# google-research/big_vision

Hardware: NVIDIA H100
Metric: siglip_vit_b16_pairs_per_sec (higher is better)
Workload: dtype bf16

## Files before the change

big_vision_b200/csrc/common.cuh:

```cuda
#pragma once
#include <cuda.h>
#include <cuda_bf16.h>
#include <cuda_runtime.h>
#include <stdint.h>
#include "wgmma.cuh"

namespace bv {

typedef __nv_bfloat16 bf16;

enum : int { DT_F32 = 0, DT_BF16 = 1 };

__device__ __forceinline__ uint32_t smem_u32(const void* p) {
  return static_cast<uint32_t>(__cvta_generic_to_shared(p));
}
__device__ __forceinline__ uint32_t lane_id() { return threadIdx.x & 31; }

__device__ __forceinline__ uint32_t pin_reg(uint32_t v) {
  return __shfl_sync(0xffffffffu, v, static_cast<int>(threadIdx.x & 31));
}
__device__ __forceinline__ int pin_reg(int v) { return static_cast<int>(pin_reg(static_cast<uint32_t>(v))); }
__device__ __forceinline__ float pin_reg(float v) { return __uint_as_float(pin_reg(__float_as_uint(v))); }
template <typename T>
__device__ __forceinline__ T* pin_reg(T* v) {
  const unsigned long long u = reinterpret_cast<unsigned long long>(v);
  const uint32_t lo = pin_reg(static_cast<uint32_t>(u)), hi = pin_reg(static_cast<uint32_t>(u >> 32));
  return reinterpret_cast<T*>((static_cast<unsigned long long>(hi) << 32) | lo);
}

__device__ __forceinline__ float warp_sum(float v) {
#pragma unroll
  for (int o = 16; o > 0; o >>= 1) v += __shfl_xor_sync(0xffffffffu, v, o);
  return v;
}
__device__ __forceinline__ float warp_max(float v) {
#pragma unroll
  for (int o = 16; o > 0; o >>= 1) v = fmaxf(v, __shfl_xor_sync(0xffffffffu, v, o));
  return v;
}

__device__ __forceinline__ uint32_t pack_bf16(float lo, float hi) {
  __nv_bfloat162 v = __floats2bfloat162_rn(lo, hi);
  return *reinterpret_cast<uint32_t*>(&v);
}
__device__ __forceinline__ uint4 ld_nc_na(const uint4* p) {
  uint4 v;
  asm volatile("ld.global.nc.L1::no_allocate.v4.u32 {%0, %1, %2, %3}, [%4];"
               : "=r"(v.x), "=r"(v.y), "=r"(v.z), "=r"(v.w) : "l"(p));
  return v;
}
__device__ __forceinline__ float bf16_lo(uint32_t v) { return __uint_as_float(v << 16); }
__device__ __forceinline__ float bf16_hi(uint32_t v) { return __uint_as_float(v & 0xffff0000u); }
__device__ __forceinline__ float round_bf16(float x) {
  return __bfloat162float(__float2bfloat16_rn(x));
}

__device__ __forceinline__ float tanh_fast(float x) {
  float y;
  asm("tanh.approx.f32 %0, %1;" : "=f"(y) : "f"(x));
  return y;
}
__device__ __forceinline__ float gelu_tanh(float x) {
  const float k0 = 0.7978845608028654f, k1 = 0.044715f;
  float u = k0 * (x + k1 * x * x * x);
  float t = 1.0f - 2.0f / (1.0f + __expf(2.0f * u));
  return 0.5f * x * (1.0f + t);
}
__device__ __forceinline__ float gelu_tanh_grad(float x) {
  const float k0 = 0.7978845608028654f, k1 = 0.044715f;
  float x2 = x * x;
  float u = k0 * (x + k1 * x * x2);
  float t = 1.0f - 2.0f / (1.0f + __expf(2.0f * u));
  float du = k0 * (1.0f + 3.0f * k1 * x2);
  return 0.5f * (1.0f + t) + 0.5f * x * (1.0f - t * t) * du;
}

__device__ __forceinline__ float gelu_tanh_fast(float x) {
  const float k0 = 0.7978845608028654f, k01 = 0.7978845608028654f * 0.044715f;
  const float t = tanh_fast(x * fmaf(k01, x * x, k0));
  const float h = 0.5f * x;
  return fmaf(h, t, h);
}
__device__ __forceinline__ float gelu_tanh_grad_fast(float x) {
  const float k0 = 0.7978845608028654f, k01 = 0.7978845608028654f * 0.044715f;
  const float x2 = x * x;
  const float t = tanh_fast(x * fmaf(k01, x2, k0));
  const float du = fmaf(3.0f * k01, x2, k0);
  return fmaf(0.5f * x * fmaf(-t, t, 1.0f), du, fmaf(0.5f, t, 0.5f));
}

__device__ __forceinline__ void mbar_init(uint32_t bar, uint32_t count) {
  asm volatile("mbarrier.init.shared::cta.b64 [%0], %1;" ::"r"(bar), "r"(count) : "memory");
}
__device__ __forceinline__ void mbar_expect_tx(uint32_t bar, uint32_t bytes) {
  asm volatile("mbarrier.arrive.expect_tx.shared::cta.b64 _, [%0], %1;" ::"r"(bar), "r"(bytes)
               : "memory");
}
__device__ __forceinline__ void mbar_arrive(uint32_t bar) {
  asm volatile("mbarrier.arrive.shared::cta.b64 _, [%0];" ::"r"(bar) : "memory");
}
__device__ __forceinline__ void mbar_wait(uint32_t bar, uint32_t parity) {
  uint32_t ok;
  do {
#ifdef BV_MBAR_SUSPEND_NS
    asm volatile(
        "{\n"
        ".reg .pred p;\n"
        "mbarrier.try_wait.parity.shared::cta.b64 p, [%1], %2, %3;\n"
        "selp.u32 %0, 1, 0, p;\n"
        "}\n"
        : "=r"(ok)
        : "r"(bar), "r"(parity), "r"(static_cast<uint32_t>(BV_MBAR_SUSPEND_NS))
        : "memory");
#else
    asm volatile(
        "{\n"
        ".reg .pred p;\n"
        "mbarrier.try_wait.parity.shared::cta.b64 p, [%1], %2;\n"
        "selp.u32 %0, 1, 0, p;\n"
        "}\n"
        : "=r"(ok)
        : "r"(bar), "r"(parity)
        : "memory");
#endif
  } while (!ok);
}
__device__ __forceinline__ bool mbar_test(uint32_t bar, uint32_t parity) {
  uint32_t ok;
  asm volatile(
      "{\n"
      ".reg .pred p;\n"
      "mbarrier.test_wait.parity.shared::cta.b64 p, [%1], %2;\n"
      "selp.u32 %0, 1, 0, p;\n"
      "}\n"
      : "=r"(ok)
      : "r"(bar), "r"(parity)
      : "memory");
  return ok != 0;
}
__device__ __forceinline__ bool elect_one() {
  uint32_t pred;
  asm volatile(
      "{\n"
      ".reg .pred P;\n"
      "elect.sync _|P, 0xffffffff;\n"
      "selp.u32 %0, 1, 0, P;\n"
      "}\n"
      : "=r"(pred));
  return pred != 0;
}
__device__ __forceinline__ void fence_barrier_init() {
  asm volatile("fence.mbarrier_init.release.cluster;" ::: "memory");
}
__device__ __forceinline__ void fence_proxy_async() {
  asm volatile("fence.proxy.async.shared::cta;" ::: "memory");
}
__device__ __forceinline__ void named_bar_sync(uint32_t id, uint32_t nthreads) {
  asm volatile("bar.sync %0, %1;" ::"r"(id), "r"(nthreads) : "memory");
}

__device__ __forceinline__ void tma_prefetch_desc(const CUtensorMap* m) {
  asm volatile("prefetch.tensormap [%0];" ::"l"(reinterpret_cast<uint64_t>(m)) : "memory");
}
__device__ __forceinline__ void tma_load_2d(uint32_t dst, const CUtensorMap* m, uint32_t bar,
                                            int c0, int c1) {
  asm volatile(
      "cp.async.bulk.tensor.2d.shared::cluster.global.mbarrier::complete_tx::bytes"
      " [%0], [%1, {%3, %4}], [%2];"
      ::"r"(dst), "l"(reinterpret_cast<uint64_t>(m)), "r"(bar), "r"(c0), "r"(c1)
      : "memory");
}
__device__ __forceinline__ void tma_load_3d(uint32_t dst, const CUtensorMap* m, uint32_t bar,
                                            int c0, int c1, int c2) {
  asm volatile(
      "cp.async.bulk.tensor.3d.shared::cluster.global.mbarrier::complete_tx::bytes"
      " [%0], [%1, {%3, %4, %5}], [%2];"
      ::"r"(dst), "l"(reinterpret_cast<uint64_t>(m)), "r"(bar), "r"(c0), "r"(c1), "r"(c2)
      : "memory");
}
__device__ __forceinline__ void tma_load_4d(uint32_t dst, const CUtensorMap* m, uint32_t bar,
                                            int c0, int c1, int c2, int c3) {
  asm volatile(
      "cp.async.bulk.tensor.4d.shared::cluster.global.mbarrier::complete_tx::bytes"
      " [%0], [%1, {%3, %4, %5, %6}], [%2];"
      ::"r"(dst), "l"(reinterpret_cast<uint64_t>(m)), "r"(bar), "r"(c0), "r"(c1), "r"(c2), "r"(c3)
      : "memory");
}
__device__ __forceinline__ void tma_store_2d(const CUtensorMap* m, uint32_t src, int c0, int c1) {
  asm volatile("cp.async.bulk.tensor.2d.global.shared::cta.bulk_group [%0, {%2, %3}], [%1];"
               ::"l"(reinterpret_cast<uint64_t>(m)), "r"(src), "r"(c0), "r"(c1)
               : "memory");
}
__device__ __forceinline__ void tma_store_3d(const CUtensorMap* m, uint32_t src, int c0, int c1,
                                             int c2) {
  asm volatile("cp.async.bulk.tensor.3d.global.shared::cta.bulk_group [%0, {%2, %3, %4}], [%1];"
               ::"l"(reinterpret_cast<uint64_t>(m)), "r"(src), "r"(c0), "r"(c1), "r"(c2)
               : "memory");
}
__device__ __forceinline__ void tma_reduce_add_2d(const CUtensorMap* m, uint32_t src, int c0,
                                                  int c1) {
  asm volatile(
      "cp.reduce.async.bulk.tensor.2d.global.shared::cta.add.bulk_group [%0, {%2, %3}], [%1];"
      ::"l"(reinterpret_cast<uint64_t>(m)), "r"(src), "r"(c0), "r"(c1)
      : "memory");
}
__device__ __forceinline__ void tma_reduce_add_3d(const CUtensorMap* m, uint32_t src, int c0,
                                                  int c1, int c2) {
  asm volatile(
      "cp.reduce.async.bulk.tensor.3d.global.shared::cta.add.bulk_group [%0, {%2, %3, %4}], [%1];"
      ::"l"(reinterpret_cast<uint64_t>(m)), "r"(src), "r"(c0), "r"(c1), "r"(c2)
      : "memory");
}
__device__ __forceinline__ void tma_store_commit() {
  asm volatile("cp.async.bulk.commit_group;" ::: "memory");
}
template <int N>
__device__ __forceinline__ void tma_store_wait_read() {
  asm volatile("cp.async.bulk.wait_group.read %0;" ::"n"(N) : "memory");
}
template <int N>
__device__ __forceinline__ void tma_store_wait() {
  asm volatile("cp.async.bulk.wait_group %0;" ::"n"(N) : "memory");
}

}
```

big_vision_b200/csrc/gemm.cu:

```cuda
#include "common.cuh"
#include "gemm_sched.h"
#include "host_utils.h"

#include <atomic>

#include <stdlib.h>
#include <string.h>

namespace bv {

namespace {

constexpr int BM = 128;
constexpr int BK = 64;
constexpr int A_STAGE_BYTES = BM * BK * 2;
constexpr int NUM_THREADS = 384;
constexpr int SUB_BYTES = 64 * 64 * 2;

enum : int { EF_BIAS = 0, EF_GELU = 1, EF_RESID = 2, EF_DGELU = 3, EF_RESID_ROWMOD = 4, EF_GELU_ACT = 5 };
enum : int { OM_F32 = 0, OM_BF16_ADD = 1, OM_BF16_TMA = 2 };

template <int BN, int OM, int EF>
struct Cfg {
  static constexpr int B_STAGE_BYTES = BN * BK * 2;
  static constexpr int STAGE_BYTES = A_STAGE_BYTES + B_STAGE_BYTES;
  static constexpr bool AUX_TMA = OM == OM_BF16_TMA && (EF == EF_RESID || EF == EF_DGELU);
  static constexpr int OUTS = OM != OM_BF16_TMA ? 0 : (EF == EF_GELU ? 2 : 1);
  static constexpr int BUF_BYTES = OUTS * SUB_BYTES;
  static constexpr int BUFS = AUX_TMA ? BN / 64 : 2;
  static constexpr int STAGING_BYTES = 2 * BUFS * BUF_BYTES;
  static constexpr int SMEM_LIMIT = 232448 - 2048;
  static constexpr int STAGES_FIT = (SMEM_LIMIT - STAGING_BYTES) / STAGE_BYTES;
  static constexpr int STAGES = STAGES_FIT > 8 ? 8 : STAGES_FIT;
  static constexpr int STAGING_OFFSET = STAGES * STAGE_BYTES;
  static constexpr int BAR_OFFSET = STAGING_OFFSET + STAGING_BYTES;
  static constexpr int AUX_BAR = 2 * STAGES;
  static constexpr int SMEM_BYTES = BAR_OFFSET + 256 + 1024;
  static_assert(STAGES >= 3, "shared-memory budget leaves fewer than 3 stages");
  static_assert(8 * (AUX_BAR + (AUX_TMA ? 2 * BUFS : 0)) <= 256, "barriers overflow their 256 bytes");
};

struct GemmDev {
  GemmSched s;
  int M, N;
  int a_mn, b_mn;
  int reduce_out;
  float alpha;
  const float* bias;
  const bf16* aux;
  void* d; void* d2;
  long long ldd, ldd2, ldaux;
  float* colsum;
  int aux_row_mod;
};

template <int BN, int STAGES, int STAGE_BYTES, int TA, int TB, typename F>
__device__ __forceinline__ void mainloop(float (&acc)[BN / 2], uint32_t base, uint32_t bar_base, int cw,
                                         PipeState& ps, int kb0, int kb1, F&& after_first) {
  constexpr uint32_t a_lbo = TA ? 8192u : 16u, b_lbo = TB ? 8192u : 16u;
  constexpr uint32_t a_kstep = TA ? 2048u : 32u, b_kstep = TB ? 2048u : 32u;
  int prev_stage = -1;
  for (int kb = kb0; kb < kb1; ++kb) {
    mbar_wait(bar_base + 8u * ps.stage, ps.phase);
    const uint32_t a_s = base + ps.stage * STAGE_BYTES + cw * 8192;
    const uint32_t b_s = base + ps.stage * STAGE_BYTES + A_STAGE_BYTES;
    const uint64_t adesc = wgmma_desc_sw128(a_s, a_lbo, 1024u), bdesc = wgmma_desc_sw128(b_s, b_lbo, 1024u);
    wgmma_fence_regs(acc);
    wgmma_fence();
#pragma unroll
    for (int k = 0; k < BK / 16; ++k) {
      const uint64_t a = adesc + k * (a_kstep >> 4), b = bdesc + k * (b_kstep >> 4);
      const int accumulate = (kb > kb0 || k > 0) ? 1 : 0;
      if constexpr (BN == 256) wgmma_ss_n256<TA, TB>(acc, a, b, accumulate);
      else wgmma_ss_n128<TA, TB>(acc, a, b, accumulate);
    }
    wgmma_commit();
    wgmma_fence_regs(acc);
    if (kb == kb0) after_first();
    wgmma_wait<1>();
    if (prev_stage >= 0 && (threadIdx.x & 127) == 0) mbar_arrive(bar_base + 8u * (STAGES + prev_stage));
    prev_stage = ps.stage;
    ps.advance(STAGES);
  }
  wgmma_wait<0>();
  wgmma_fence_regs(acc);
  if (prev_stage >= 0 && (threadIdx.x & 127) == 0) mbar_arrive(bar_base + 8u * (STAGES + prev_stage));
}

__device__ __forceinline__ void aux_global(const GemmDev& p, int row, int col, bool pair, float& a0, float& a1) {
  const long long ar = p.aux_row_mod > 0 ? (row % p.aux_row_mod) : row;
  const bf16* ap = p.aux + ar * p.ldaux + col;
  if (pair) {
    const uint32_t q = *reinterpret_cast<const uint32_t*>(ap);
    a0 = bf16_lo(q); a1 = bf16_hi(q);
  } else {
    a0 = __bfloat162float(*ap);
    a1 = 0.f;
  }
}

template <bool OUT_F32, int EF>
__device__ __forceinline__ void epi_math(float alpha, float c0, float c1, float b0, float b1, float a0, float a1,
                                         float& v0, float& v1, float& pre0, float& pre1) {
  v0 = c0 * alpha + b0;
  v1 = c1 * alpha + b1;
  pre0 = pre1 = 0.f;
  if (EF == EF_GELU || EF == EF_GELU_ACT) {
    pre0 = round_bf16(v0); pre1 = round_bf16(v1);
    v0 = gelu_tanh_fast(pre0); v1 = gelu_tanh_fast(pre1);
  } else if (EF == EF_RESID || EF == EF_RESID_ROWMOD) {
    v0 = (OUT_F32 ? v0 : round_bf16(v0)) + a0;
    v1 = (OUT_F32 ? v1 : round_bf16(v1)) + a1;
  } else if (EF == EF_DGELU) {
    v0 *= gelu_tanh_grad_fast(a0);
    v1 *= gelu_tanh_grad_fast(a1);
  }
}


__device__ __forceinline__ void colsum_add(float* colsum, int N, float s0, float s1, int col, int lane) {
  s0 += __shfl_xor_sync(0xffffffffu, s0, 4);
  s0 += __shfl_xor_sync(0xffffffffu, s0, 8);
  s0 += __shfl_xor_sync(0xffffffffu, s0, 16);
  s1 += __shfl_xor_sync(0xffffffffu, s1, 4);
  s1 += __shfl_xor_sync(0xffffffffu, s1, 8);
  s1 += __shfl_xor_sync(0xffffffffu, s1, 16);
  if (lane < 4) {
    if (col < N) atomicAdd(colsum + col, s0);
    if (col + 1 < N) atomicAdd(colsum + col + 1, s1);
  }
}

template <int BN, bool OUT_F32, int EF>
__device__ __forceinline__ void epilogue_regs(const GemmDev& p, const float (&acc)[BN / 2], int m0, int n0,
                                              int cw, int kb0) {
  const int lane = threadIdx.x & 31, warp = (threadIdx.x >> 5) & 3;
  const int row0 = m0 + cw * 64 + warp * 16 + (lane >> 2);
  const int pM = p.M, pN = p.N;
  const float alpha = p.alpha;
  const bool reduce = p.reduce_out != 0;
  const bool first = kb0 == 0;
#pragma unroll
  for (int j = 0; j < BN / 8; ++j) {
    const int col = n0 + 8 * j + 2 * (lane & 3);
    if (col >= pN) continue;
    const bool pair = col + 1 < pN;
    float b0 = 0.f, b1 = 0.f;
    if (p.bias != nullptr && first) {
      b0 = __ldg(p.bias + col);
      if (pair) b1 = __ldg(p.bias + col + 1);
    }
#pragma unroll
    for (int h = 0; h < 2; ++h) {
      const int row = row0 + 8 * h;
      if (row >= pM) continue;
      float v0, v1, pre0, pre1, a0 = 0.f, a1 = 0.f;
      if ((EF == EF_RESID && first) || EF == EF_DGELU) aux_global(p, row, col, pair, a0, a1);
      epi_math<OUT_F32, EF>(alpha, acc[4 * j + 2 * h], acc[4 * j + 2 * h + 1], b0, b1, a0, a1, v0, v1, pre0, pre1);
      if (OUT_F32) {
        float* dp = static_cast<float*>(p.d) + row * p.ldd + col;
        if (reduce) {
          atomicAdd(dp, v0);
          if (pair) atomicAdd(dp + 1, v1);
        } else if (pair) {
          *reinterpret_cast<float2*>(dp) = make_float2(v0, v1);
        } else {
          *dp = v0;
        }
      } else {
        bf16* dp = static_cast<bf16*>(p.d) + row * p.ldd + col;
        const __nv_bfloat162 o = __floats2bfloat162_rn(v0, v1);
        if (pair) atomicAdd(reinterpret_cast<__nv_bfloat162*>(dp), o);
        else atomicAdd(dp, o.x);
      }
    }
  }
}

template <int BN, int EF, int BUF_BYTES>
__device__ __forceinline__ void epilogue_tma(const GemmDev& p, const CUtensorMap* tmD, const CUtensorMap* tmD2,
                                             const float (&acc)[BN / 2], int m0, int n0, int cw, uint32_t staging,
                                             uint32_t& nstore, uint32_t aux_bar, uint32_t aux_parity) {
  constexpr bool AUX_TMA = (EF == EF_RESID || EF == EF_DGELU);
  const int lane = threadIdx.x & 31, warp = (threadIdx.x >> 5) & 3;
  const bool leader = (threadIdx.x & 127) == 0;
  const int rl0 = warp * 16 + (lane >> 2);
  const int row0 = m0 + cw * 64 + rl0;
  const int pM = p.M, pN = p.N, pN8 = p.N & ~7;
  const float alpha = p.alpha;
#pragma unroll
  for (int c = 0; c < BN / 64; ++c) {
    uint32_t buf;
    if constexpr (AUX_TMA) {
      buf = staging + c * BUF_BYTES;
      mbar_wait(aux_bar + 8u * c, aux_parity);
    } else {
      buf = staging + (nstore & 1u) * BUF_BYTES;
      if (leader) tma_store_wait_read<1>();
      named_bar_sync(1 + cw, 128);
    }
    float cs[8][2];
#pragma unroll
    for (int jj = 0; jj < 8; ++jj) {
      const int j = 8 * c + jj;
      const int col = n0 + 8 * j + 2 * (lane & 3);
      cs[jj][0] = cs[jj][1] = 0.f;
      const bool cin = col < pN, pair = col + 1 < pN;
      float b0 = 0.f, b1 = 0.f;
      if (cin && p.bias != nullptr) {
        b0 = __ldg(p.bias + col);
        if (pair) b1 = __ldg(p.bias + col + 1);
      }
#pragma unroll
      for (int h = 0; h < 2; ++h) {
        const int rl = rl0 + 8 * h, row = row0 + 8 * h;
        const uint32_t off = rl * 128 + ((jj ^ (rl & 7)) << 4) + (lane & 3) * 4;
        float v0 = 0.f, v1 = 0.f, pre0 = 0.f, pre1 = 0.f;
        const bool in = cin && row < pM;
        if (in) {
          float a0 = 0.f, a1 = 0.f;
          if constexpr (AUX_TMA) {
            uint32_t q;
            asm volatile("ld.shared.b32 %0, [%1];" : "=r"(q) : "r"(buf + off));
            a0 = bf16_lo(q); a1 = bf16_hi(q);
          } else if constexpr (EF == EF_RESID_ROWMOD) {
            aux_global(p, row, col, pair, a0, a1);
          }
          epi_math<false, EF>(alpha, acc[4 * j + 2 * h], acc[4 * j + 2 * h + 1], b0, b1, a0, a1, v0, v1, pre0, pre1);
        }
        const __nv_bfloat162 o = __floats2bfloat162_rn(v0, v1);
        if (in) {
          cs[jj][0] += __low2float(o);
          cs[jj][1] += pair ? __high2float(o) : 0.f;
        }
        asm volatile("st.shared.b32 [%0], %1;" ::"r"(buf + off), "r"(*reinterpret_cast<const uint32_t*>(&o))
                     : "memory");
        if (EF == EF_GELU) {
          const __nv_bfloat162 q = __floats2bfloat162_rn(pre0, pre1);
          asm volatile("st.shared.b32 [%0], %1;" ::"r"(buf + SUB_BYTES + off),
                       "r"(*reinterpret_cast<const uint32_t*>(&q))
                       : "memory");
        }
      }
    }
    fence_proxy_async();
    named_bar_sync(1 + cw, 128);
    if (leader) {
      if (n0 + 64 * c < pN8 && m0 + cw * 64 < pM) {
        tma_store_2d(tmD, buf, n0 + 64 * c, m0 + cw * 64);
        if (EF == EF_GELU) tma_store_2d(tmD2, buf + SUB_BYTES, n0 + 64 * c, m0 + cw * 64);
      }
      tma_store_commit();
    }
    const int tail0 = pN8 - (n0 + 64 * c);
    if (pN8 < pN && tail0 >= 0 && tail0 < 64) {
      const int t = threadIdx.x & 127, rl = t & 63, out = t >> 6;
      const int row = m0 + cw * 64 + rl;
      if (row < pM && (out == 0 || EF == EF_GELU)) {
        const uint32_t src = buf + out * SUB_BYTES + rl * 128 + (((tail0 >> 3) ^ (rl & 7)) << 4);
        uint16_t* dst = reinterpret_cast<uint16_t*>(out ? p.d2 : p.d) + row * (out ? p.ldd2 : p.ldd) + pN8;
#pragma unroll 1
        for (int e = 0; e < pN - pN8; ++e) {
          uint16_t u;
          asm volatile("ld.shared.u16 %0, [%1];" : "=h"(u) : "r"(src + 2 * e));
          dst[e] = u;
        }
      }
      named_bar_sync(1 + cw, 128);
    }
    if (!AUX_TMA) ++nstore;
    if (p.colsum != nullptr) {
#pragma unroll
      for (int jj = 0; jj < 8; ++jj)
        colsum_add(p.colsum, pN, cs[jj][0], cs[jj][1], n0 + 8 * (8 * c + jj) + 2 * (lane & 3), lane);
    }
  }
}

template <int BN>
__device__ __forceinline__ void issue_aux_loads(const CUtensorMap* tmAux, int M, int N, int m0, int n0, int cw,
                                                uint32_t staging, uint32_t aux_bar) {
  tma_store_wait_read<0>();
#pragma unroll
  for (int c = 0; c < BN / 64; ++c) {
    const uint32_t bar = aux_bar + 8u * c;
    if (n0 + 64 * c < N && m0 + cw * 64 < M) {
      mbar_expect_tx(bar, SUB_BYTES);
      tma_load_2d(staging + c * SUB_BYTES, tmAux, bar, n0 + 64 * c, m0 + cw * 64);
    } else {
      mbar_arrive(bar);
    }
  }
}

template <int BN, int OM, int EF>
__global__ void __launch_bounds__(NUM_THREADS, 1)
gemm_kernel(const __grid_constant__ CUtensorMap tmA, const __grid_constant__ CUtensorMap tmB,
            const __grid_constant__ CUtensorMap tmD, const __grid_constant__ CUtensorMap tmD2,
            const __grid_constant__ CUtensorMap tmAux, const GemmDev p) {
  using C = Cfg<BN, OM, EF>;
  extern __shared__ uint8_t smem_raw[];
  const uint32_t raw_addr = smem_u32(smem_raw);
  const uint32_t base = (raw_addr + 1023u) & ~1023u;
  const uint32_t bar_base = base + C::BAR_OFFSET;
  auto full_bar = [&](int s) { return bar_base + 8u * s; };
  auto empty_bar = [&](int s) { return bar_base + 8u * (C::STAGES + s); };

  const int wg = __shfl_sync(0xffffffffu, static_cast<int>(threadIdx.x >> 7), 0);
  const int units = p.s.units;

  if (threadIdx.x == 0) {
    tma_prefetch_desc(&tmA);
    tma_prefetch_desc(&tmB);
    if (C::AUX_TMA) tma_prefetch_desc(&tmAux);
    for (int s = 0; s < C::STAGES; ++s) {
      mbar_init(full_bar(s), 1);
      mbar_init(empty_bar(s), 2);
    }
    if (C::AUX_TMA) {
      for (int b = 0; b < 2 * C::BUFS; ++b) mbar_init(bar_base + 8u * (C::AUX_BAR + b), 1);
    }
    fence_barrier_init();
  }
  __syncthreads();

  if (wg == 0) {
    asm volatile("setmaxnreg.dec.sync.aligned.u32 40;");
    if (threadIdx.x == 0) {
      PipeState ps;
      for (int u = blockIdx.x; u < units; u += gridDim.x) {
        const WorkUnit w = gemm_work_unit(p.s, u, BM, BN);
        for (int kb = w.kb0; kb < w.kb1; ++kb) {
          mbar_wait(empty_bar(ps.stage), ps.phase ^ 1u);
          const uint32_t a_s = base + ps.stage * C::STAGE_BYTES;
          const uint32_t b_s = a_s + A_STAGE_BYTES;
          const uint32_t fb = full_bar(ps.stage);
          mbar_expect_tx(fb, C::STAGE_BYTES);
          const int k0 = kb * BK;
          if (p.a_mn) {
#pragma unroll
            for (int j = 0; j < BM / 64; ++j) tma_load_2d(a_s + j * 8192, &tmA, fb, w.m0 + 64 * j, k0);
          } else {
            tma_load_2d(a_s, &tmA, fb, k0, w.m0);
          }
          if (p.b_mn) {
#pragma unroll
            for (int j = 0; j < BN / 64; ++j) tma_load_2d(b_s + j * 8192, &tmB, fb, w.n0 + 64 * j, k0);
          } else {
            tma_load_2d(b_s, &tmB, fb, k0, w.n0);
          }
          ps.advance(C::STAGES);
        }
      }
    }
    return;
  }

  asm volatile("setmaxnreg.inc.sync.aligned.u32 232;");
  const int cw = wg - 1;
  const uint32_t staging = base + C::STAGING_OFFSET + cw * C::BUFS * C::BUF_BYTES;
  const uint32_t aux_bar = bar_base + 8u * (C::AUX_BAR + cw * C::BUFS);
  const bool leader = (threadIdx.x & 127) == 0;
  uint32_t nstore = 0, nunit = 0;
  PipeState ps;
  constexpr int S = C::STAGES, SB = C::STAGE_BYTES;
  for (int u = blockIdx.x; u < units; u += gridDim.x, ++nunit) {
    const WorkUnit w = gemm_work_unit(p.s, u, BM, BN);
    auto after_first = [&]() {
      if constexpr (C::AUX_TMA) {
        if (leader) issue_aux_loads<BN>(&tmAux, p.M, p.N, w.m0, w.n0, cw, staging, aux_bar);
      }
    };
    float acc[BN / 2];
    if (p.a_mn) {
      if (p.b_mn) mainloop<BN, S, SB, 1, 1>(acc, base, bar_base, cw, ps, w.kb0, w.kb1, after_first);
      else mainloop<BN, S, SB, 1, 0>(acc, base, bar_base, cw, ps, w.kb0, w.kb1, after_first);
    } else {
      if (p.b_mn) mainloop<BN, S, SB, 0, 1>(acc, base, bar_base, cw, ps, w.kb0, w.kb1, after_first);
      else mainloop<BN, S, SB, 0, 0>(acc, base, bar_base, cw, ps, w.kb0, w.kb1, after_first);
    }

    if constexpr (OM == OM_BF16_TMA)
      epilogue_tma<BN, EF, C::BUF_BYTES>(p, &tmD, &tmD2, acc, w.m0, w.n0, cw, staging, nstore, aux_bar, nunit & 1u);
    else epilogue_regs<BN, OM == OM_F32, EF>(p, acc, w.m0, w.n0, cw, w.kb0);
  }
  if (OM == OM_BF16_TMA && (threadIdx.x & 127) == 0) tma_store_wait<0>();
}

template <int BN, int OM, int EF>
int launch_cfg(const bv_gemm_args& g, cudaStream_t stream) {
  using C = Cfg<BN, OM, EF>;
  CUtensorMap tmA, tmB, tmD, tmD2, tmAux;
  int rc;
  const CUtensorMapDataType bf = CU_TENSOR_MAP_DATA_TYPE_BFLOAT16;
  if (g.a_mn) rc = make_tmap_2d(&tmA, bf, g.A, g.M, g.K, g.lda * 2, 64, 64);
  else        rc = make_tmap_2d(&tmA, bf, g.A, g.K, g.M, g.lda * 2, 64, BM);
  if (rc) return rc;
  if (g.b_mn) rc = make_tmap_2d(&tmB, bf, g.B, g.N, g.K, g.ldb * 2, 64, 64);
  else        rc = make_tmap_2d(&tmB, bf, g.B, g.K, g.N, g.ldb * 2, 64, BN);
  if (rc) return rc;

  GemmDev p;
  const long long tiles = ((g.M + BM - 1) / BM) * ((g.N + BN - 1) / BN);
  if (tiles * ((g.K + BK - 1) / BK) > 0x7fffffffLL) { set_error("bv_gemm: problem too large"); return BV_ERR_INVALID; }
  if (!gemm_make_sched(g.M, g.N, g.K, BM, BN, BK, g.splits, g.reduce_out != 0, num_sms(), &p.s)) {
    set_error("bv_gemm: split-K requires reduce_out=1");
    return BV_ERR_INVALID;
  }
  p.M = (int)g.M; p.N = (int)g.N;
  p.a_mn = g.a_mn; p.b_mn = g.b_mn; p.reduce_out = g.reduce_out;
  p.alpha = g.alpha;
  p.bias = g.epilogue == BV_EPI_NONE ? nullptr : g.bias;
  p.colsum = g.colsum;
  p.aux = reinterpret_cast<const bf16*>(g.aux);
  p.ldaux = g.ldaux;
  p.aux_row_mod = g.aux_row_mod;
  p.d = g.D; p.d2 = g.D2;
  p.ldd = g.ldd; p.ldd2 = g.ldd2;
  memset(&tmD, 0, sizeof(tmD));
  memset(&tmD2, 0, sizeof(tmD2));
  memset(&tmAux, 0, sizeof(tmAux));
  const long long n8 = g.N & ~7LL;
  if (OM == OM_BF16_TMA && n8 > 0) {
    rc = make_tmap_2d(&tmD, bf, g.D, n8, g.M, g.ldd * 2, 64, 64);
    if (rc) return rc;
    if (EF == EF_GELU) {
      rc = make_tmap_2d(&tmD2, bf, g.D2, n8, g.M, g.ldd2 * 2, 64, 64);
      if (rc) return rc;
    }
  }
  if (C::AUX_TMA) {
    rc = make_tmap_2d(&tmAux, bf, g.aux, g.N, g.M, g.ldaux * 2, 64, 64);
    if (rc) return rc;
  }

  auto kern = gemm_kernel<BN, OM, EF>;
  static std::atomic<bool> attr_set[64];
  int dev = 0;
  if (cudaGetDevice(&dev) != cudaSuccess || dev < 0 || dev >= 64) dev = -1;
  if (dev < 0 || !attr_set[dev].load(std::memory_order_acquire)) {
    rc = check_cuda(cudaFuncSetAttribute(kern, cudaFuncAttributeMaxDynamicSharedMemorySize, C::SMEM_BYTES),
                    "cudaFuncSetAttribute(gemm)");
    if (rc) return rc;
    if (dev >= 0) attr_set[dev].store(true, std::memory_order_release);
  }
  const int grid = p.s.units < num_sms() ? p.s.units : num_sms();
  kern<<<grid, NUM_THREADS, C::SMEM_BYTES, stream>>>(tmA, tmB, tmD, tmD2, tmAux, p);
  return check_cuda(cudaGetLastError(), "gemm_kernel launch");
}

template <int BN>
int dispatch_epi(const bv_gemm_args& g, cudaStream_t s) {
  const bool f32 = (g.out_dtype == DT_F32), add = !f32 && g.reduce_out;
  switch (g.epilogue) {
    case BV_EPI_NONE:
    case BV_EPI_BIAS:
      return f32 ? launch_cfg<BN, OM_F32, EF_BIAS>(g, s)
                 : add ? launch_cfg<128, OM_BF16_ADD, EF_BIAS>(g, s) : launch_cfg<BN, OM_BF16_TMA, EF_BIAS>(g, s);
    case BV_EPI_BIAS_RESID:
      if (f32) return launch_cfg<BN, OM_F32, EF_RESID>(g, s);
      if (add) return launch_cfg<128, OM_BF16_ADD, EF_RESID>(g, s);
      return g.aux_row_mod > 0 ? launch_cfg<BN, OM_BF16_TMA, EF_RESID_ROWMOD>(g, s)
                               : launch_cfg<BN, OM_BF16_TMA, EF_RESID>(g, s);
    case BV_EPI_BIAS_GELU:
      return launch_cfg<BN, OM_BF16_TMA, EF_GELU>(g, s);
    case BV_EPI_BIAS_GELU_ACT:
      return launch_cfg<BN, OM_BF16_TMA, EF_GELU_ACT>(g, s);
    case BV_EPI_DGELU:
      if (f32) { set_error("bv_gemm: DGELU epilogue writes bf16"); return BV_ERR_INVALID; }
      if (g.aux_row_mod > 0) { set_error("bv_gemm: DGELU takes a row-aligned aux"); return BV_ERR_INVALID; }
      return add ? launch_cfg<128, OM_BF16_ADD, EF_DGELU>(g, s) : launch_cfg<BN, OM_BF16_TMA, EF_DGELU>(g, s);
  }
  set_error("bv_gemm: bad epilogue %d", g.epilogue);
  return BV_ERR_INVALID;
}

}
}

extern "C" {

int bv_gemm(const bv_gemm_args* args, void* stream) {
  using namespace bv;
  const cudaStream_t s = static_cast<cudaStream_t>(stream);
  if (!args) { set_error("bv_gemm: null args"); return BV_ERR_INVALID; }
  const bv_gemm_args& g = *args;
  if (g.M <= 0 || g.N <= 0 || g.K <= 0) { set_error("bv_gemm: empty problem"); return BV_ERR_INVALID; }
  if (g.out_dtype == DT_BF16 && ((reinterpret_cast<uintptr_t>(g.D) & 15) || (g.ldd % 8))) {
    set_error("bv_gemm: bf16 output must be 16B aligned with ldd %% 8 == 0"); return BV_ERR_INVALID;
  }
  if (g.out_dtype == DT_F32 && ((reinterpret_cast<uintptr_t>(g.D) & 7) || (g.ldd % 2))) {
    set_error("bv_gemm: fp32 output must be 8B aligned with an even ldd"); return BV_ERR_INVALID;
  }
  if (g.M > 0x7fffffffLL || g.N > 0x7fffffffLL || g.K > 0x7fffffffLL) {
    set_error("bv_gemm: dimension exceeds int32"); return BV_ERR_INVALID;
  }
  if (g.epilogue < BV_EPI_NONE || g.epilogue > BV_EPI_BIAS_GELU_ACT) {
    set_error("bv_gemm: bad epilogue %d", g.epilogue); return BV_ERR_INVALID;
  }
  if ((g.epilogue == BV_EPI_BIAS_RESID || g.epilogue == BV_EPI_DGELU) && g.aux == nullptr) {
    set_error("bv_gemm: epilogue %d needs aux", g.epilogue); return BV_ERR_INVALID;
  }
  if (g.aux != nullptr && ((reinterpret_cast<uintptr_t>(g.aux) & 15) || (g.ldaux % 8))) {
    set_error("bv_gemm: aux must be 16B aligned with ldaux %% 8 == 0"); return BV_ERR_INVALID;
  }
  if (g.bias != nullptr && (reinterpret_cast<uintptr_t>(g.bias) & 15)) {
    set_error("bv_gemm: bias must be 16B aligned"); return BV_ERR_INVALID;
  }
  if (g.epilogue == BV_EPI_BIAS_GELU && (g.out_dtype != DT_BF16 || g.D2 == nullptr || g.reduce_out)) {
    set_error("bv_gemm: BIAS_GELU needs bf16 output, D2 and no reduce"); return BV_ERR_INVALID;
  }
  if (g.epilogue == BV_EPI_BIAS_GELU && ((reinterpret_cast<uintptr_t>(g.D2) & 15) || (g.ldd2 % 8))) {
    set_error("bv_gemm: D2 must be 16B aligned with ldd2 %% 8 == 0"); return BV_ERR_INVALID;
  }
  if (g.epilogue == BV_EPI_BIAS_GELU_ACT && (g.out_dtype != DT_BF16 || g.reduce_out)) {
    set_error("bv_gemm: BIAS_GELU_ACT needs bf16 output and no reduce"); return BV_ERR_INVALID;
  }
  if (g.out_dtype != DT_F32 && g.out_dtype != DT_BF16) { set_error("bv_gemm: bad out dtype"); return BV_ERR_INVALID; }
  if (g.colsum != nullptr && (g.out_dtype != DT_BF16 || g.reduce_out)) {
    set_error("bv_gemm: colsum needs a plain bf16 output"); return BV_ERR_INVALID;
  }
  int bn = g.block_n;
  if (bn == 0) bn = (g.N > 128) ? 256 : 128;
  if (bn == 256) return dispatch_epi<256>(g, s);
  if (bn == 128) return dispatch_epi<128>(g, s);
  set_error("bv_gemm: block_n must be 0, 128 or 256");
  return BV_ERR_INVALID;
}

}
```

Measured before the change: 2765.

## Add ping-pong consumer schedule for TMA-stored GEMMs with small K

Adds a ping-pong mode where the two consumer warpgroups alternate whole 128x128 work units instead of splitting rows of one unit. Each warpgroup computes both 64-row halves, and named barriers order the mainloops so one group's epilogue overlaps the other's MMA. It is selected for bf16 TMA-output GEMMs with K<=1024, such as the ViT-B projections. The cost is a doubled accumulator register footprint, extra staging buffers for aux loads, and fixed BN=128 tiles in place of the chosen BN.

New measurement: 2825 (median of 6 runs). 1.02x the previous value.

```diff
diff --git a/big_vision_b200/csrc/common.cuh b/big_vision_b200/csrc/common.cuh
--- a/big_vision_b200/csrc/common.cuh
+++ b/big_vision_b200/csrc/common.cuh
@@ -158,6 +158,9 @@
 __device__ __forceinline__ void named_bar_sync(uint32_t id, uint32_t nthreads) {
   asm volatile("bar.sync %0, %1;" ::"r"(id), "r"(nthreads) : "memory");
 }
+__device__ __forceinline__ void named_bar_arrive(uint32_t id, uint32_t nthreads) {
+  asm volatile("bar.arrive %0, %1;" ::"r"(id), "r"(nthreads) : "memory");
+}
 
 __device__ __forceinline__ void tma_prefetch_desc(const CUtensorMap* m) {
   asm volatile("prefetch.tensormap [%0];" ::"l"(reinterpret_cast<uint64_t>(m)) : "memory");
diff --git a/big_vision_b200/csrc/gemm.cu b/big_vision_b200/csrc/gemm.cu
--- a/big_vision_b200/csrc/gemm.cu
+++ b/big_vision_b200/csrc/gemm.cu
@@ -16,18 +16,20 @@
 constexpr int A_STAGE_BYTES = BM * BK * 2;
 constexpr int NUM_THREADS = 384;
 constexpr int SUB_BYTES = 64 * 64 * 2;
+constexpr uint32_t ORDER_BAR = 3;
+constexpr long long PINGPONG_MAX_K = 1024;
 
 enum : int { EF_BIAS = 0, EF_GELU = 1, EF_RESID = 2, EF_DGELU = 3, EF_RESID_ROWMOD = 4, EF_GELU_ACT = 5 };
 enum : int { OM_F32 = 0, OM_BF16_ADD = 1, OM_BF16_TMA = 2 };
 
-template <int BN, int OM, int EF>
+template <int BN, int OM, int EF, bool PP>
 struct Cfg {
   static constexpr int B_STAGE_BYTES = BN * BK * 2;
   static constexpr int STAGE_BYTES = A_STAGE_BYTES + B_STAGE_BYTES;
   static constexpr bool AUX_TMA = OM == OM_BF16_TMA && (EF == EF_RESID || EF == EF_DGELU);
   static constexpr int OUTS = OM != OM_BF16_TMA ? 0 : (EF == EF_GELU ? 2 : 1);
   static constexpr int BUF_BYTES = OUTS * SUB_BYTES;
-  static constexpr int BUFS = AUX_TMA ? BN / 64 : 2;
+  static constexpr int BUFS = AUX_TMA ? (PP ? 2 : 1) * BN / 64 : 2;
   static constexpr int STAGING_BYTES = 2 * BUFS * BUF_BYTES;
   static constexpr int SMEM_LIMIT = 232448 - 2048;
   static constexpr int STAGES_FIT = (SMEM_LIMIT - STAGING_BYTES) / STAGE_BYTES;
@@ -54,36 +56,43 @@
   int aux_row_mod;
 };
 
-template <int BN, int STAGES, int STAGE_BYTES, int TA, int TB, typename F>
-__device__ __forceinline__ void mainloop(float (&acc)[BN / 2], uint32_t base, uint32_t bar_base, int cw,
-                                         PipeState& ps, int kb0, int kb1, F&& after_first) {
+template <int BN, int H, int STAGES, int STAGE_BYTES, int TA, int TB, typename F, typename G>
+__device__ __forceinline__ void mainloop(float (&acc)[H][BN / 2], uint32_t base, uint32_t bar_base, uint32_t a_off,
+                                         PipeState& ps, int kb0, int kb1, F&& after_first, G&& after_issue) {
   constexpr uint32_t a_lbo = TA ? 8192u : 16u, b_lbo = TB ? 8192u : 16u;
   constexpr uint32_t a_kstep = TA ? 2048u : 32u, b_kstep = TB ? 2048u : 32u;
   int prev_stage = -1;
   for (int kb = kb0; kb < kb1; ++kb) {
     mbar_wait(bar_base + 8u * ps.stage, ps.phase);
-    const uint32_t a_s = base + ps.stage * STAGE_BYTES + cw * 8192;
+    const uint32_t a_s = base + ps.stage * STAGE_BYTES + a_off;
     const uint32_t b_s = base + ps.stage * STAGE_BYTES + A_STAGE_BYTES;
     const uint64_t adesc = wgmma_desc_sw128(a_s, a_lbo, 1024u), bdesc = wgmma_desc_sw128(b_s, b_lbo, 1024u);
-    wgmma_fence_regs(acc);
+#pragma unroll
+    for (int h = 0; h < H; ++h) wgmma_fence_regs(acc[h]);
     wgmma_fence();
 #pragma unroll
     for (int k = 0; k < BK / 16; ++k) {
       const uint64_t a = adesc + k * (a_kstep >> 4), b = bdesc + k * (b_kstep >> 4);
       const int accumulate = (kb > kb0 || k > 0) ? 1 : 0;
-      if constexpr (BN == 256) wgmma_ss_n256<TA, TB>(acc, a, b, accumulate);
-      else wgmma_ss_n128<TA, TB>(acc, a, b, accumulate);
+#pragma unroll
+      for (int h = 0; h < H; ++h) {
+        if constexpr (BN == 256) wgmma_ss_n256<TA, TB>(acc[h], a + h * (8192 >> 4), b, accumulate);
+        else wgmma_ss_n128<TA, TB>(acc[h], a + h * (8192 >> 4), b, accumulate);
+      }
     }
     wgmma_commit();
-    wgmma_fence_regs(acc);
+#pragma unroll
+    for (int h = 0; h < H; ++h) wgmma_fence_regs(acc[h]);
     if (kb == kb0) after_first();
     wgmma_wait<1>();
     if (prev_stage >= 0 && (threadIdx.x & 127) == 0) mbar_arrive(bar_base + 8u * (STAGES + prev_stage));
     prev_stage = ps.stage;
     ps.advance(STAGES);
   }
+  after_issue();
   wgmma_wait<0>();
-  wgmma_fence_regs(acc);
+#pragma unroll
+  for (int h = 0; h < H; ++h) wgmma_fence_regs(acc[h]);
   if (prev_stage >= 0 && (threadIdx.x & 127) == 0) mbar_arrive(bar_base + 8u * (STAGES + prev_stage));
 }
 
@@ -179,13 +188,13 @@
 
 template <int BN, int EF, int BUF_BYTES>
 __device__ __forceinline__ void epilogue_tma(const GemmDev& p, const CUtensorMap* tmD, const CUtensorMap* tmD2,
-                                             const float (&acc)[BN / 2], int m0, int n0, int cw, uint32_t staging,
+                                             const float (&acc)[BN / 2], int r0, int n0, int cw, uint32_t staging,
                                              uint32_t& nstore, uint32_t aux_bar, uint32_t aux_parity) {
   constexpr bool AUX_TMA = (EF == EF_RESID || EF == EF_DGELU);
   const int lane = threadIdx.x & 31, warp = (threadIdx.x >> 5) & 3;
   const bool leader = (threadIdx.x & 127) == 0;
   const int rl0 = warp * 16 + (lane >> 2);
-  const int row0 = m0 + cw * 64 + rl0;
+  const int row0 = r0 + rl0;
   const int pM = p.M, pN = p.N, pN8 = p.N & ~7;
   const float alpha = p.alpha;
 #pragma unroll
@@ -246,16 +255,16 @@
     fence_proxy_async();
     named_bar_sync(1 + cw, 128);
     if (leader) {
-      if (n0 + 64 * c < pN8 && m0 + cw * 64 < pM) {
-        tma_store_2d(tmD, buf, n0 + 64 * c, m0 + cw * 64);
-        if (EF == EF_GELU) tma_store_2d(tmD2, buf + SUB_BYTES, n0 + 64 * c, m0 + cw * 64);
+      if (n0 + 64 * c < pN8 && r0 < pM) {
+        tma_store_2d(tmD, buf, n0 + 64 * c, r0);
+        if (EF == EF_GELU) tma_store_2d(tmD2, buf + SUB_BYTES, n0 + 64 * c, r0);
       }
       tma_store_commit();
     }
     const int tail0 = pN8 - (n0 + 64 * c);
     if (pN8 < pN && tail0 >= 0 && tail0 < 64) {
       const int t = threadIdx.x & 127, rl = t & 63, out = t >> 6;
-      const int row = m0 + cw * 64 + rl;
+      const int row = r0 + rl;
       if (row < pM && (out == 0 || EF == EF_GELU)) {
         const uint32_t src = buf + out * SUB_BYTES + rl * 128 + (((tail0 >> 3) ^ (rl & 7)) << 4);
         uint16_t* dst = reinterpret_cast<uint16_t*>(out ? p.d2 : p.d) + row * (out ? p.ldd2 : p.ldd) + pN8;
@@ -278,27 +287,28 @@
 }
 
 template <int BN>
-__device__ __forceinline__ void issue_aux_loads(const CUtensorMap* tmAux, int M, int N, int m0, int n0, int cw,
+__device__ __forceinline__ void issue_aux_loads(const CUtensorMap* tmAux, int M, int N, int r0, int n0,
                                                 uint32_t staging, uint32_t aux_bar) {
   tma_store_wait_read<0>();
 #pragma unroll
   for (int c = 0; c < BN / 64; ++c) {
     const uint32_t bar = aux_bar + 8u * c;
-    if (n0 + 64 * c < N && m0 + cw * 64 < M) {
+    if (n0 + 64 * c < N && r0 < M) {
       mbar_expect_tx(bar, SUB_BYTES);
-      tma_load_2d(staging + c * SUB_BYTES, tmAux, bar, n0 + 64 * c, m0 + cw * 64);
+      tma_load_2d(staging + c * SUB_BYTES, tmAux, bar, n0 + 64 * c, r0);
     } else {
       mbar_arrive(bar);
     }
   }
 }
 
-template <int BN, int OM, int EF>
+template <int BN, int OM, int EF, bool PP>
 __global__ void __launch_bounds__(NUM_THREADS, 1)
 gemm_kernel(const __grid_constant__ CUtensorMap tmA, const __grid_constant__ CUtensorMap tmB,
             const __grid_constant__ CUtensorMap tmD, const __grid_constant__ CUtensorMap tmD2,
             const __grid_constant__ CUtensorMap tmAux, const GemmDev p) {
-  using C = Cfg<BN, OM, EF>;
+  using C = Cfg<BN, OM, EF, PP>;
+  static_assert(!PP || (BN == 128 && OM == OM_BF16_TMA), "ping-pong units are 128 x 128 with TMA-stored outputs");
   extern __shared__ uint8_t smem_raw[];
   const uint32_t raw_addr = smem_u32(smem_raw);
   const uint32_t base = (raw_addr + 1023u) & ~1023u;
@@ -315,7 +325,7 @@
     if (C::AUX_TMA) tma_prefetch_desc(&tmAux);
     for (int s = 0; s < C::STAGES; ++s) {
       mbar_init(full_bar(s), 1);
-      mbar_init(empty_bar(s), 2);
+      mbar_init(empty_bar(s), PP ? 1 : 2);
     }
     if (C::AUX_TMA) {
       for (int b = 0; b < 2 * C::BUFS; ++b) mbar_init(bar_base + 8u * (C::AUX_BAR + b), 1);
@@ -357,6 +367,7 @@
   }
 
   asm volatile("setmaxnreg.inc.sync.aligned.u32 232;");
+  constexpr int H = PP ? 2 : 1;
   const int cw = wg - 1;
   const uint32_t staging = base + C::STAGING_OFFSET + cw * C::BUFS * C::BUF_BYTES;
   const uint32_t aux_bar = bar_base + 8u * (C::AUX_BAR + cw * C::BUFS);
@@ -364,32 +375,56 @@
   uint32_t nstore = 0, nunit = 0;
   PipeState ps;
   constexpr int S = C::STAGES, SB = C::STAGE_BYTES;
-  for (int u = blockIdx.x; u < units; u += gridDim.x, ++nunit) {
+  int i = 0;
+  for (int u = blockIdx.x; u < units; u += gridDim.x, ++i) {
     const WorkUnit w = gemm_work_unit(p.s, u, BM, BN);
+    if (PP && (i & 1) != cw) {
+      for (int kb = w.kb0; kb < w.kb1; ++kb) ps.advance(S);
+      continue;
+    }
+    if (PP && i > 0) named_bar_sync(ORDER_BAR + cw, 256);
+    const bool has_next = units - u > static_cast<int>(gridDim.x);
+    const int r0 = w.m0 + (PP ? 0 : 64 * cw);
     auto after_first = [&]() {
       if constexpr (C::AUX_TMA) {
-        if (leader) issue_aux_loads<BN>(&tmAux, p.M, p.N, w.m0, w.n0, cw, staging, aux_bar);
+        if (leader) {
+#pragma unroll
+          for (int h = 0; h < H; ++h)
+            issue_aux_loads<BN>(&tmAux, p.M, p.N, r0 + 64 * h, w.n0, staging + h * (BN / 64) * SUB_BYTES,
+                                aux_bar + 8u * h * (BN / 64));
+        }
       }
     };
-    float acc[BN / 2];
+    auto after_issue = [&]() {
+      if (PP && has_next) named_bar_arrive(ORDER_BAR + (cw ^ 1), 256);
+    };
+    float acc[H][BN / 2];
+    const uint32_t a_off = PP ? 0u : cw * 8192u;
     if (p.a_mn) {
-      if (p.b_mn) mainloop<BN, S, SB, 1, 1>(acc, base, bar_base, cw, ps, w.kb0, w.kb1, after_first);
-      else mainloop<BN, S, SB, 1, 0>(acc, base, bar_base, cw, ps, w.kb0, w.kb1, after_first);
+      if (p.b_mn) mainloop<BN, H, S, SB, 1, 1>(acc, base, bar_base, a_off, ps, w.kb0, w.kb1, after_first, after_issue);
+      else mainloop<BN, H, S, SB, 1, 0>(acc, base, bar_base, a_off, ps, w.kb0, w.kb1, after_first, after_issue);
     } else {
-      if (p.b_mn) mainloop<BN, S, SB, 0, 1>(acc, base, bar_base, cw, ps, w.kb0, w.kb1, after_first);
-      else mainloop<BN, S, SB, 0, 0>(acc, base, bar_base, cw, ps, w.kb0, w.kb1, after_first);
-    }
-
-    if constexpr (OM == OM_BF16_TMA)
-      epilogue_tma<BN, EF, C::BUF_BYTES>(p, &tmD, &tmD2, acc, w.m0, w.n0, cw, staging, nstore, aux_bar, nunit & 1u);
-    else epilogue_regs<BN, OM == OM_F32, EF>(p, acc, w.m0, w.n0, cw, w.kb0);
+      if (p.b_mn) mainloop<BN, H, S, SB, 0, 1>(acc, base, bar_base, a_off, ps, w.kb0, w.kb1, after_first, after_issue);
+      else mainloop<BN, H, S, SB, 0, 0>(acc, base, bar_base, a_off, ps, w.kb0, w.kb1, after_first, after_issue);
+    }
+
+    if constexpr (OM == OM_BF16_TMA) {
+#pragma unroll
+      for (int h = 0; h < H; ++h)
+        epilogue_tma<BN, EF, C::BUF_BYTES>(p, &tmD, &tmD2, acc[h], r0 + 64 * h, w.n0, cw,
+                                           staging + (C::AUX_TMA ? h * (BN / 64) * C::BUF_BYTES : 0), nstore,
+                                           aux_bar + (C::AUX_TMA ? 8u * h * (BN / 64) : 0u), nunit & 1u);
+    } else {
+      epilogue_regs<BN, OM == OM_F32, EF>(p, acc[0], w.m0, w.n0, cw, w.kb0);
+    }
+    ++nunit;
   }
   if (OM == OM_BF16_TMA && (threadIdx.x & 127) == 0) tma_store_wait<0>();
 }
 
-template <int BN, int OM, int EF>
+template <int BN, int OM, int EF, bool PP = false>
 int launch_cfg(const bv_gemm_args& g, cudaStream_t stream) {
-  using C = Cfg<BN, OM, EF>;
+  using C = Cfg<BN, OM, EF, PP>;
   CUtensorMap tmA, tmB, tmD, tmD2, tmAux;
   int rc;
   const CUtensorMapDataType bf = CU_TENSOR_MAP_DATA_TYPE_BFLOAT16;
@@ -434,7 +469,7 @@
     if (rc) return rc;
   }
 
-  auto kern = gemm_kernel<BN, OM, EF>;
+  auto kern = gemm_kernel<BN, OM, EF, PP>;
   static std::atomic<bool> attr_set[64];
   int dev = 0;
   if (cudaGetDevice(&dev) != cudaSuccess || dev < 0 || dev >= 64) dev = -1;
@@ -449,6 +484,11 @@
   return check_cuda(cudaGetLastError(), "gemm_kernel launch");
 }
 
+template <int BN, int EF>
+int launch_tma(const bv_gemm_args& g, cudaStream_t s) {
+  return g.K <= PINGPONG_MAX_K ? launch_cfg<128, OM_BF16_TMA, EF, true>(g, s) : launch_cfg<BN, OM_BF16_TMA, EF>(g, s);
+}
+
 template <int BN>
 int dispatch_epi(const bv_gemm_args& g, cudaStream_t s) {
   const bool f32 = (g.out_dtype == DT_F32), add = !f32 && g.reduce_out;
@@ -456,20 +496,19 @@
     case BV_EPI_NONE:
     case BV_EPI_BIAS:
       return f32 ? launch_cfg<BN, OM_F32, EF_BIAS>(g, s)
-                 : add ? launch_cfg<128, OM_BF16_ADD, EF_BIAS>(g, s) : launch_cfg<BN, OM_BF16_TMA, EF_BIAS>(g, s);
+                 : add ? launch_cfg<128, OM_BF16_ADD, EF_BIAS>(g, s) : launch_tma<BN, EF_BIAS>(g, s);
     case BV_EPI_BIAS_RESID:
       if (f32) return launch_cfg<BN, OM_F32, EF_RESID>(g, s);
       if (add) return launch_cfg<128, OM_BF16_ADD, EF_RESID>(g, s);
-      return g.aux_row_mod > 0 ? launch_cfg<BN, OM_BF16_TMA, EF_RESID_ROWMOD>(g, s)
-                               : launch_cfg<BN, OM_BF16_TMA, EF_RESID>(g, s);
+      return g.aux_row_mod > 0 ? launch_tma<BN, EF_RESID_ROWMOD>(g, s) : launch_tma<BN, EF_RESID>(g, s);
     case BV_EPI_BIAS_GELU:
-      return launch_cfg<BN, OM_BF16_TMA, EF_GELU>(g, s);
+      return launch_tma<BN, EF_GELU>(g, s);
     case BV_EPI_BIAS_GELU_ACT:
-      return launch_cfg<BN, OM_BF16_TMA, EF_GELU_ACT>(g, s);
+      return launch_tma<BN, EF_GELU_ACT>(g, s);
     case BV_EPI_DGELU:
       if (f32) { set_error("bv_gemm: DGELU epilogue writes bf16"); return BV_ERR_INVALID; }
       if (g.aux_row_mod > 0) { set_error("bv_gemm: DGELU takes a row-aligned aux"); return BV_ERR_INVALID; }
-      return add ? launch_cfg<128, OM_BF16_ADD, EF_DGELU>(g, s) : launch_cfg<BN, OM_BF16_TMA, EF_DGELU>(g, s);
+      return add ? launch_cfg<128, OM_BF16_ADD, EF_DGELU>(g, s) : launch_tma<BN, EF_DGELU>(g, s);
   }
   set_error("bv_gemm: bad epilogue %d", g.epilogue);
   return BV_ERR_INVALID;
```
